# bioinformatics-centre/kaiju

Measured on NVIDIA H100. Metric: reads/sec (150 bp paired, MEM mode, synth-viruses .fmi), higher is better.
Workload: dtype int64

## Files before the change

kaiju_b200/csrc/kj_build.h:

```cpp
#pragma once

#define KJ_BLD_THREADS 256
struct KjBuildLcode { uint8_t v[256]; };

template <int RB>
__global__ void __launch_bounds__(KJ_BLD_THREADS) kj_bld_count(const uint8_t* __restrict__ bwt, const __grid_constant__ KjBuildLcode lc, uint64_t n, uint32_t rep, int alen,
                                                                uint32_t* __restrict__ tile_counts) {
    __shared__ uint32_t tot[KJ_MAX_ALEN];
    __shared__ uint8_t lcs[256];
    __shared__ uint8_t cnt[KJ_MAX_ALEN * KJ_BLD_THREADS];
    if (threadIdx.x < KJ_MAX_ALEN) tot[threadIdx.x] = 0;
    lcs[threadIdx.x] = lc.v[threadIdx.x];
    for (int a = 0; a < KJ_MAX_ALEN; a++) cnt[a * KJ_BLD_THREADS + threadIdx.x] = 0;
    __syncthreads();
    const uint64_t tile_rows = (uint64_t)KJ_BLD_THREADS * RB, start = (uint64_t)blockIdx.x * tile_rows;
    for (uint32_t i = threadIdx.x; i < tile_rows; i += KJ_BLD_THREADS) {
        const uint64_t row = start + i;
        if (row < n) cnt[(uint32_t)lcs[bwt[rep == 1 ? row : row / rep]] * KJ_BLD_THREADS + threadIdx.x]++;
    }
    for (int a = 0; a < alen; a++) {
        uint32_t v = cnt[a * KJ_BLD_THREADS + threadIdx.x];
        for (int m = 16; m > 0; m >>= 1) v += __shfl_xor_sync(0xffffffffu, v, m);
        if ((threadIdx.x & 31) == 0 && v) atomicAdd(&tot[a], v);
    }
// ... 40 lines not shown
            #pragma unroll
            for (int x = 0; x < 16; x++) {
                const uint32_t m = __vcmpeq4(mine[q * 16 + x], a4) & 0x01010101u;
                bits |= (uint64_t)((m * 0x01020408u) >> 24) << (4 * x);
            }
            w[q] = bits; c += (uint32_t)__popcll(bits);
        }
        uint32_t x = c;
        for (int d = 1; d < 32; d <<= 1) { const uint32_t o = __shfl_up_sync(0xffffffffu, x, d); if (lane >= (uint32_t)d) x += o; }
        if (lane == 31) wsum[wid] = x;
        __syncthreads();
        uint32_t base = 0;
        for (uint32_t k = 0; k < wid; k++) base += wsum[k];
        __syncthreads();
        if (b < nb) {
            uint64_t hdr = Cdev[a] + tile_prefix[(uint64_t)blockIdx.x * KJ_MAX_ALEN + a] + (uint64_t)(base + x - c);
            uint64_t* rec = rank + ((uint64_t)a * nb + b) * RW;
            if (RW == 2) { *(ulonglong2*)rec = make_ulonglong2(hdr, w[0]); }
            else {
                const uint64_t p1 = (uint64_t)__popcll(w[0]), p2 = p1 + (uint64_t)__popcll(w[RB / 64 > 1 ? 1 : 0]);
                hdr = (hdr & KJ_CNT_MASK) | (p1 << KJ_P1_SHIFT) | (p2 << KJ_P2_SHIFT);
                *(ulonglong2*)rec = make_ulonglong2(hdr, w[0]);
                *(ulonglong2*)(rec + 2) = make_ulonglong2(w[RB / 64 > 1 ? 1 : 0], w[RB / 64 > 2 ? 2 : 0]);
            }
        }
    }
}
__global__ void kj_bld_letters(const uint8_t* __restrict__ bwt, const __grid_constant__ KjBuildLcode lc, uint64_t n, uint32_t rep, uint64_t nwords, uint64_t* __restrict__ letters) {
    __shared__ uint8_t lcs[256];
    lcs[threadIdx.x] = lc.v[threadIdx.x];
    __syncthreads();
    for (uint64_t wd = (uint64_t)blockIdx.x * blockDim.x + threadIdx.x; wd < nwords; wd += (uint64_t)gridDim.x * blockDim.x) {
        uint64_t v = 0;
        for (int t = 0; t < KJ_LETTERS_PER_WORD; t++) { const uint64_t row = wd * KJ_LETTERS_PER_WORD + t; if (row < n) v |= (uint64_t)lcs[bwt[rep == 1 ? row : row / rep]] << (5 * t); }
        letters[wd] = v;
    }
}
__global__ void kj_bld_sa_tax(const uint8_t* __restrict__ sa, uint64_t n_entries, uint64_t first, int nbytes, int pbits, uint32_t nseq, const uint32_t* __restrict__ seq_tax,
                              uint32_t* __restrict__ sa_tax, uint32_t* __restrict__ err) {
    for (uint64_t e = (uint64_t)blockIdx.x * blockDim.x + threadIdx.x; e < n_entries; e += (uint64_t)gridDim.x * blockDim.x) {
        const uint8_t* p = sa + e * (uint64_t)nbytes; uint64_t val = 0;
        for (int b = 0; b < nbytes; b++) val = (val << 8) + p[b];
        const uint64_t seq = val >> pbits;
        if (seq >= nseq) { atomicOr(err, 64u); continue; }
        sa_tax[first + e] = seq_tax[seq];
    }
}
template <class IdxT>
__global__ void kj_bld_sa_tax_scaled(const KjDevIndex* __restrict__ base_ix, uint64_t n_entries, int64_t bias, int exp, uint64_t n_rows, uint32_t rep, uint32_t* __restrict__ sa_tax) {
    for (uint64_t e = (uint64_t)blockIdx.x * blockDim.x + threadIdx.x; e < n_entries; e += (uint64_t)gridDim.x * blockDim.x) {
        const uint64_t k = (uint64_t)((int64_t)e + bias) << exp;
        sa_tax[e] = k < n_rows ? kj_sa_taxon<IdxT>(*base_ix, k / rep) : KJ_TAX_BAD;
    }
}
__global__ void kj_bld_repeat_u32(const uint32_t* __restrict__ src, uint64_t n_out, uint32_t rep, uint32_t* __restrict__ dst) {
    for (uint64_t i = (uint64_t)blockIdx.x * blockDim.x + threadIdx.x; i < n_out; i += (uint64_t)gridDim.x * blockDim.x) dst[i] = src[i / rep];
}
template <class IdxT>
static __device__ __forceinline__ uint64_t kj_bld_rank(const KjDevIndex& ix, uint32_t c, uint64_t k) {
    uint64_t v = (uint64_t)kj_rank<IdxT>(ix, c, (IdxT)k);
    if (k >= ix.quirk_lo) v -= ix.quirk_d[c];
    return v;
}
template <class IdxT>
__global__ void kj_bld_quirk(const KjDevIndex* __restrict__ ix, uint64_t k, uint64_t* __restrict__ quirk_d) {
    const uint32_t a = threadIdx.x;
    if (a < (uint32_t)ix->alen) quirk_d[a] = (uint64_t)kj_rank<IdxT>(*ix, a, (IdxT)k) - ix->C[a];
}
template <class IdxT>
__global__ void kj_bld_kmer_level(const KjDevIndex* __restrict__ ix, const KjKmer* __restrict__ cur, uint64_t n_cur, KjKmer* __restrict__ nxt) {
    for (uint64_t t = (uint64_t)blockIdx.x * blockDim.x + threadIdx.x; t < n_cur * 20u; t += (uint64_t)gridDim.x * blockDim.x) {
        const KjKmer iv = cur[t / 20u]; const uint32_t a = (uint32_t)(t % 20u); KjKmer o; o.lo = 0; o.hi = 0;
        if (iv.lo < iv.hi) { o.lo = kj_bld_rank<IdxT>(*ix, a + 1u, iv.lo); o.hi = kj_bld_rank<IdxT>(*ix, a + 1u, iv.hi); if (o.lo >= o.hi) { o.lo = 0; o.hi = 0; } }
        nxt[t] = o;
    }
}
__global__ void kj_bld_kmer_narrow(const KjKmer* __restrict__ src, uint64_t n, KjKmer32* __restrict__ dst) {
    for (uint64_t t = (uint64_t)blockIdx.x * blockDim.x + threadIdx.x; t < n; t += (uint64_t)gridDim.x * blockDim.x) { dst[t].lo = (uint32_t)src[t].lo; dst[t].hi = (uint32_t)src[t].hi; }
}

static int kj_bld_upload(void* d, const void* h, size_t bytes) {
    const size_t CH = (size_t)1 << 30;
    for (size_t o = 0; o < bytes; o += CH) CK(cudaMemcpy((char*)d + o, (const char*)h + o, std::min(CH, bytes - o), cudaMemcpyHostToDevice));
    return KJ_OK;
}

static int kj_device_build(kj_ctx* c, const kj_index_view& v, const uint8_t lcode[256], uint32_t rep, const kj_ctx* base, uint64_t& tot) {
    KjHostIndex& H = c->H; const int alen = H.alen; const uint64_t n = H.bwtlen, nb = H.nb; const int wide = H.wide;
    const uint32_t RB = kj_rank_rows(wide), RW = kj_rank_words(wide);
    KjBuildLcode lc; memcpy(lc.v, lcode, 256);
    const int grid_big = c->sm_count * 16;
    KjDevBuf bwt; int rc = bwt.grow((size_t)v.bwtlen); if (rc) return rc;
    const uint8_t* d_bwt = bwt.as<uint8_t>();
    if ((rc = kj_bld_upload(bwt.p, v.bwt, (size_t)v.bwtlen))) return rc;
    const uint64_t ntiles = (nb + KJ_BLD_THREADS - 1) / KJ_BLD_THREADS;
    if (ntiles >= (1ull << 31)) { kj_err() = "index too large"; return KJ_ERR_UNSUPPORTED; }
    KjDevBuf tc, tp, small;
    if ((rc = tc.grow(ntiles * KJ_MAX_ALEN * 4)) || (rc = tp.grow(ntiles * KJ_MAX_ALEN * 8)) || (rc = small.grow(3 * KJ_MAX_ALEN * 8 + 64))) return rc;
    uint32_t* d_tc = tc.as<uint32_t>(); uint64_t* d_tp = tp.as<uint64_t>();
    uint64_t* d_tot = small.as<uint64_t>(); uint64_t* d_C = d_tot + KJ_MAX_ALEN + 1;
    if (wide) kj_bld_count<KJ_RANK_ROWS_WIDE><<<(unsigned)ntiles, KJ_BLD_THREADS>>>(d_bwt, lc, n, rep, alen, d_tc);
    else kj_bld_count<KJ_RANK_ROWS_NARROW><<<(unsigned)ntiles, KJ_BLD_THREADS>>>(d_bwt, lc, n, rep, alen, d_tc);
    kj_bld_scan_tiles<<<1, 32 * KJ_MAX_ALEN>>>(d_tc, ntiles, d_tp, d_tot);
    CK(cudaGetLastError());
    uint64_t tots[KJ_MAX_ALEN]; CK(cudaMemcpy(tots, d_tot, sizeof tots, cudaMemcpyDeviceToHost));
    H.C[0] = 0; for (int a = 0; a < alen; a++) H.C[a + 1] = H.C[a] + tots[a];
// ... 39 lines not shown
            const uint64_t m = std::min(CHE, n_sa - e0);
            CK(cudaMemcpy(sa.p, v.sa + e0 * (uint64_t)v.nbytes, (size_t)m * (size_t)v.nbytes, cudaMemcpyHostToDevice));
            kj_bld_sa_tax<<<grid_big, 256>>>(sa.as<uint8_t>(), m, e0, v.nbytes, v.pbits, (uint32_t)v.nseq, c->seq_tax.as<uint32_t>(), c->sa_tax.as<uint32_t>(), d_err);
            if (c->sa_acc.p) kj_bld_sa_tax<<<grid_big, 256>>>(sa.as<uint8_t>(), m, e0, v.nbytes, v.pbits, (uint32_t)v.nseq, c->seq_acc.as<uint32_t>(), c->sa_acc.as<uint32_t>(), d_err);
            CK(cudaGetLastError()); CK(cudaDeviceSynchronize()); c->launches++;
        }
        uint32_t e = 0; CK(cudaMemcpy(&e, d_err, 4, cudaMemcpyDeviceToHost));
        if (e & 64u) { CK(cudaMemset(d_err, 0, 4)); kj_err() = "corrupt suffix array (sequence number out of range)"; return KJ_ERR_IO; }
    } else {
        const int64_t last = (int64_t)((n - 1) >> H.sa_exp) - H.sa_bias;
        n_sa = last >= 0 ? (uint64_t)last + 1 : 0;
        if ((rc = c->sa_tax.grow(std::max<size_t>(n_sa * 4, 16)))) return rc;
        tot += std::max<size_t>(n_sa * 4, 16);
        if (base->H.wide) kj_bld_sa_tax_scaled<uint64_t><<<grid_big, 256>>>(base->ix.as<KjDevIndex>(), n_sa, H.sa_bias, H.sa_exp, n, rep, c->sa_tax.as<uint32_t>());
        else kj_bld_sa_tax_scaled<uint32_t><<<grid_big, 256>>>(base->ix.as<KjDevIndex>(), n_sa, H.sa_bias, H.sa_exp, n, rep, c->sa_tax.as<uint32_t>());
        CK(cudaGetLastError()); CK(cudaDeviceSynchronize()); c->launches++;
    }
    c->n_sa = n_sa;
    return KJ_OK;
}

static int kj_device_build_kmer(kj_ctx* c, int k, uint64_t& tot, KjDevBuf& dst, int& k_out) {
    KjHostIndex& H = c->H; const int wide = H.wide; const KjDevIndex* ix = c->ix.as<KjDevIndex>();
    if (H.quirk_lo != ~0ull && &dst == &c->kmer) {
        if (wide) kj_bld_quirk<uint64_t><<<1, 32>>>(ix, H.bwtlen - 65536ull, c->quirk.as<uint64_t>()); else kj_bld_quirk<uint32_t><<<1, 32>>>(ix, H.bwtlen - 65536ull, c->quirk.as<uint64_t>());
        CK(cudaGetLastError()); CK(cudaMemcpy(H.quirk_d, c->quirk.p, sizeof H.quirk_d, cudaMemcpyDeviceToHost)); c->launches++;
    }
    k_out = 0;
    if (k < 2 || k > 7 || H.alen != 21) return KJ_OK;
    uint64_t n_final = 1; for (int d = 0; d < k; d++) n_final *= 20;
    { size_t fr = 0, to = 0; CK(cudaMemGetInfo(&fr, &to));
      while (k > 2 && (double)n_final * (2.0 * sizeof(KjKmer) + sizeof(KjKmer32)) > 0.8 * (double)fr) { k--; n_final /= 20; } }
    KjDevBuf a, b; int rc;
    if ((rc = a.grow(n_final * sizeof(KjKmer))) || (rc = b.grow(n_final * sizeof(KjKmer)))) return rc;
    std::vector<KjKmer> first(20); for (uint32_t l = 0; l < 20; l++) { first[l].lo = H.C[l + 1]; first[l].hi = H.C[l + 2]; }
    CK(cudaMemcpy(a.p, first.data(), 20 * sizeof(KjKmer), cudaMemcpyHostToDevice));
    uint64_t n_cur = 20;
    for (int d = 1; d < k; d++) {
        const unsigned g = (unsigned)std::min<uint64_t>((n_cur * 20 + 255) / 256, (uint64_t)c->sm_count * 32);
        if (wide) kj_bld_kmer_level<uint64_t><<<g, 256>>>(ix, a.as<KjKmer>(), n_cur, b.as<KjKmer>()); else kj_bld_kmer_level<uint32_t><<<g, 256>>>(ix, a.as<KjKmer>(), n_cur, b.as<KjKmer>());
        CK(cudaGetLastError()); c->launches++;
        std::swap(a, b); n_cur *= 20;
    }
    if (wide) { dst = std::move(a); tot += n_final * sizeof(KjKmer); }
    else {
        if ((rc = dst.grow(n_final * sizeof(KjKmer32)))) return rc;
        tot += n_final * sizeof(KjKmer32);
        kj_bld_kmer_narrow<<<c->sm_count * 8, 256>>>(a.as<KjKmer>(), n_final, dst.as<KjKmer32>()); CK(cudaGetLastError()); c->launches++;
    }
    CK(cudaDeviceSynchronize());
    k_out = k;
    return KJ_OK;
}
```

kaiju_b200/csrc/kj_core.h:

```cpp
#pragma once
#include "kj_warp.h"
#include "kj_layout.h"

#define KJ_SEG_CAP(max_frag) ((max_frag) / 4u + 8u)
struct KjKept { uint64_t lo; uint32_t len; uint32_t aux; };

struct KjSmemLayout {
    uint32_t qkey_off, qpay_off, kept_off, res_off, res2_off, pre_off, ids_off, qord_off, aa_off, aa_stride, frag_off, hflag_off,
             segcnt_off, seghist_off, accs_off, total, segs_off;
#if defined(KJ_EMU)
    uint32_t guard[16], nguard;
#endif
};
#if defined(KJ_EMU)
#define KJ_GUARD(L, o) { (L).guard[(L).nguard++] = (o); (o) += 64u; }
#else
#define KJ_GUARD(L, o)
#endif
static KJ_HD uint32_t kj_align(uint32_t x, uint32_t a) { return (x + a - 1) / a * a; }
static KJ_HD KjSmemLayout kj_smem_layout(const KjRunParams& p) {
    KjSmemLayout L; uint32_t o = 0;
#if defined(KJ_EMU)
    L.nguard = 0;
#endif
// ... 41 lines not shown
};
static KJ_DEV void kj_flag_error(KjWarpCtx& cx, uint32_t bit) {
#if defined(KJ_EMU)
    *cx.err |= bit;
#else
    atomicOr(cx.err, bit);
#endif
}

static KJ_DEV uint64_t kj_ld64(const void* p) {
#if defined(KJ_EMU)
    return *(const uint64_t*)p;
#else
    uint64_t v; asm volatile("ld.global.nc.u64 %0, [%1];" : "=l"(v) : "l"(p)); return v;
#endif
}
static KJ_DEV void kj_ld128(const void* p, uint64_t& a, uint64_t& b) {
#if defined(KJ_EMU)
    a = ((const uint64_t*)p)[0]; b = ((const uint64_t*)p)[1];
#else
    asm volatile("ld.global.nc.v2.u64 {%0, %1}, [%2];" : "=l"(a), "=l"(b) : "l"(p));
#endif
}
template <class IdxT>
static KJ_DEV IdxT kj_rank_at(const uint64_t* base, IdxT k) {
    if (sizeof(IdxT) == 4) {
        uint64_t h, wd; kj_ld128(base + 2u * (size_t)((uint32_t)k >> 6), h, wd);
        return (IdxT)((uint32_t)h + (uint32_t)kj_popcll(wd & ((1ull << ((uint32_t)k & 63u)) - 1ull)));
    }
    const uint32_t q = (uint32_t)((uint64_t)k >> 6), blk = q / 3u, wi = q - 3u * blk, bit = (uint32_t)k & 63u;
    const uint64_t* rec = base + 4u * (size_t)blk;
    const uint64_t hdr = kj_ld64(rec);
    const uint64_t ww = kj_ld64(rec + 1u + wi);
    const uint32_t pc = (uint32_t)kj_popcll(ww & ((1ull << bit) - 1ull));
    const uint32_t add = wi == 0 ? 0u : ((uint32_t)(hdr >> (32u + 8u * wi)) & 0xffu);
    return (IdxT)((hdr & KJ_CNT_MASK) + (uint64_t)(add + pc));
}
static KJ_DEV const uint64_t* kj_letter_base(const KjDevIndex& ix, uint32_t c) { return ix.rank_base[c]; }
template <class IdxT>
static KJ_DEV IdxT kj_rank(const KjDevIndex& ix, uint32_t c, IdxT k) { return kj_rank_at<IdxT>(kj_letter_base(ix, c), k); }
template <class IdxT>
static KJ_DEV bool kj_update_si(const KjDevIndex& ix, uint32_t c, IdxT& lo, IdxT& hi) {
    const uint64_t* base = kj_letter_base(ix, c);
    IdxT nlo = kj_rank_at<IdxT>(base, lo), nhi = kj_rank_at<IdxT>(base, hi);
    if (sizeof(IdxT) == 8) { if (hi >= (IdxT)ix.quirk_lo) { const IdxT d = (IdxT)ix.quirk_d[c]; nhi -= d; if (lo >= (IdxT)ix.quirk_lo) nlo -= d; } }
    if (nlo >= nhi) return false;
    lo = nlo; hi = nhi; return true;
}
static KJ_DEV int kj_hibit64(uint64_t x) { uint32_t h = (uint32_t)(x >> 32); return h ? 63 - kj_clz(h) : 31 - kj_clz((uint32_t)x); }
static KJ_DEV uint32_t kj_letter(const KjDevIndex& ix, uint64_t k) {
    uint64_t wd = k / KJ_LETTERS_PER_WORD; uint32_t s = (uint32_t)(k - wd * KJ_LETTERS_PER_WORD) * 5u;
    return (uint32_t)(ix.letters[wd] >> s) & 31u;
}
template <class IdxT>
static KJ_DEV uint64_t kj_sa_locate(const KjDevIndex& ix, uint64_t k, bool& is_seq) {
    uint32_t c = 1;
    KJ_ROLLED
    while (c != 0 && (k & ix.sa_check)) { c = kj_letter(ix, k); const bool q = k >= ix.quirk_lo; k = (uint64_t)kj_rank<IdxT>(ix, c, (IdxT)k); if (q) k -= ix.quirk_d[c]; }
    is_seq = c == 0;
    return is_seq ? k : (uint64_t)((int64_t)(k >> ix.sa_exp) - ix.sa_bias);
}
template <class IdxT>
static KJ_DEV uint32_t kj_sa_taxon(const KjDevIndex& ix, uint64_t k) {
    bool is_seq; const uint64_t e = kj_sa_locate<IdxT>(ix, k, is_seq);
    return is_seq ? ix.seq_tax[e] : ix.sa_tax[e];
}

#define KJ_PHASE_A_LETTERS 9
#define KJ_ST_OPEN 0
#define KJ_ST_EXACT 1
#define KJ_ST_KDEAD 2
template <class IdxT> struct KjChain { IdxT lo, hi; int i; int st; };
#if defined(KJ_EMU)
struct KjEmuStats { unsigned long long rounds, round_steps, lane_steps, chains, blocks, lookaheads, pops_frag, pops_var, var_steps, var_pushed; };
extern thread_local KjEmuStats kj_emu_stats;
#endif

template <class IdxT>
static KJ_DEV void kj_chain_start(const KjDevIndex& ix, const uint8_t* frag, int j, uint32_t Lmin, KjChain<IdxT>& ch) {
    const int k = ix.kmer_k; int i = j; int budget = KJ_PHASE_A_LETTERS - 1;
    ch.st = KJ_ST_OPEN;
    if (k > 0 && j >= k && Lmin >= (uint32_t)k) {
        uint32_t idx = 0;
        KJ_ROLLED
        for (int t = 0; t < k; t++) idx = idx * 20u + (uint32_t)(frag[j - t] - 1u);
        IdxT lo, hi;
        if (sizeof(IdxT) == 4) { const KjKmer32 e = ((const KjKmer32*)ix.kmer)[idx]; lo = (IdxT)e.lo; hi = (IdxT)e.hi; }
        else { const KjKmer e = ((const KjKmer*)ix.kmer)[idx]; lo = (IdxT)e.lo; hi = (IdxT)e.hi; }
        if (lo >= hi) { ch.lo = 0; ch.hi = 0; ch.i = j + 1; ch.st = KJ_ST_KDEAD; return; }
        ch.lo = lo; ch.hi = hi; i = j - k + 1; budget = KJ_PHASE_A_LETTERS - k;
    } else {
        const uint32_t c = frag[j]; ch.lo = (IdxT)ix.C[c]; ch.hi = (IdxT)ix.C[c + 1];
    }
    KJ_ROLLED
    while (i > 0 && budget > 0) { if (!kj_update_si<IdxT>(ix, frag[i - 1], ch.lo, ch.hi)) { ch.st = KJ_ST_EXACT; break; } i--; budget--; }
    if (i == 0) ch.st = KJ_ST_EXACT;
    ch.i = i;
}
template <class IdxT>
static KJ_DEV void kj_chain_finish(const KjDevIndex& ix, const uint8_t* frag, KjChain<IdxT>& ch) {
    int i = ch.i;
    KJ_ROLLED
    while (i > 0) { if (!kj_update_si<IdxT>(ix, frag[i - 1], ch.lo, ch.hi)) break; i--; }
    ch.i = i; ch.st = KJ_ST_EXACT;
}
template <class IdxT>
static KJ_DEV void kj_finish_selected(const Warp& w, const KjDevIndex& ix, const uint8_t* frag, bool sel, KjChain<IdxT>& ch) {
#if defined(KJ_EMU)
    const int i0 = ch.i;
#endif
    if (sel) kj_chain_finish<IdxT>(ix, frag, ch);
    w.sync();
#if defined(KJ_EMU)
    { const uint32_t st = sel ? (uint32_t)(i0 - ch.i) + 1u : 0u; const uint32_t mx = warp_max_u32(w, st); const uint32_t nsel = (uint32_t)kj_popc(w.ballot(sel));
      uint32_t sum = st; for (int m = 16; m > 0; m >>= 1) sum += w.shfl_xor(sum, m);
      if (w.lane == 0) { kj_emu_stats.rounds++; kj_emu_stats.round_steps += mx; kj_emu_stats.lane_steps += sum; kj_emu_stats.chains += nsel; } }
#endif
}

template <class IdxT>
static KJ_DEV int kj_chain_lbval(const KjChain<IdxT>& ch, int j, int kk) { return ch.st == KJ_ST_EXACT ? ch.i : (j - kk + 2 > 0 ? j - kk + 2 : 0); }
template <class IdxT>
static KJ_DEV int kj_chain_lb(const Warp& w, const KjChain<IdxT>& ch, bool ran, int j, int kk, int lb_ext) {
    const uint32_t inf = w.ballot(ran && ch.st != KJ_ST_OPEN);
    const uint32_t below = w.lane < 31 ? inf & ~((2u << w.lane) - 1u) : 0u;
    const int v = w.shfl(kj_chain_lbval<IdxT>(ch, j, kk), below ? kj_ffs(below) - 1 : 0);
    return below ? v : lb_ext;
}
template <class IdxT>
// ... 417 lines not shown
        }
    }
    return nsegs;
}
KJ_NOINLINE int kj_seg_regions(const KjSegArgs A, int n) {
    KjSeg* segs = A.segs;
    int ns = kj_seg_level<0>(A, 0, n, segs, 0);
    A.w.sync();
    if (ns > 1) {
        if (A.w.lane == 0) {
            int cur = ns - 1, nx = cur - 1;
            KJ_ROLLED
            while (nx >= 0) {
                if (segs[cur].begin - segs[nx].end - 1 < 0) {
                    if (segs[cur].end < segs[nx].end) segs[cur].end = segs[nx].end;
                    if (segs[cur].begin > segs[nx].begin) segs[cur].begin = segs[nx].begin;
                    segs[nx].begin = -1;
                } else cur = nx;
                nx--;
            }
            int o = 0;
            KJ_ROLLED
            for (int t = 0; t < ns; t++) if (segs[t].begin >= 0) segs[o++] = segs[t];
            segs[ns].begin = o;
        }
        A.w.sync();
        ns = segs[ns].begin;
        A.w.sync();
    }
    return ns;
}
static KJ_DEV int kj_seg(KjWarpCtx& cx, int n, const bool compact) {
    if (n < KJ_SEG_WINDOW) return 0;
    if (!kj_seg_flags(cx, n, compact)) return 0;
    KjSegArgs A; A.w = cx.w; A.frag = cx.smem + cx.L.frag_off; A.hf = cx.smem + cx.L.hflag_off; A.segs = (KjSeg*)(cx.smem + cx.L.segs_off);
    A.scratch = cx.smem + cx.L.segcnt_off; A.lnf = cx.ix->lnfact; A.cap = (int)KJ_SEG_CAP(cx.rp->max_frag); A.err = cx.err;
    return kj_seg_regions(A, n);
}

static KJ_DEV KjKept* kj_kept_ptr(KjWarpCtx& cx, uint32_t idx) {
    if (idx < cx.rp->kept_cap_smem) return (KjKept*)(cx.smem + cx.L.kept_off) + idx;
    uint32_t s = idx - cx.rp->kept_cap_smem;
    if (s >= cx.rp->scratch_entries) { kj_flag_error(cx, 2u); s = cx.rp->scratch_entries - 1; }
    return cx.spill + s;
}

struct KjIdsArgs { Warp w; const KjDevIndex* ix; const KjKept* kept_smem; const KjKept* spill; uint32_t kept_cap, spill_cap; uint32_t* ids; uint32_t* accs; };
template <class IdxT>
KJ_NOINLINE uint64_t kj_ids_and_lca_fn(const KjIdsArgs A, uint32_t nkept) {
    const Warp& w = A.w; const KjDevIndex& ix = *A.ix;
    uint32_t* ids = A.ids;
    uint32_t nids = 0, nacc = 0;
    uint32_t* accs = A.accs;
    KJ_ROLLED
    for (uint32_t e = 0; e < nkept && nids <= 20; e++) {
        const uint32_t se = e - A.kept_cap;
        const KjKept kk = e < A.kept_cap ? A.kept_smem[e] : A.spill[se < A.spill_cap ? se : A.spill_cap - 1];
        KJ_ROLLED
        for (uint32_t base = 0; base < kk.len && nids <= 20; base += 32) {
            uint32_t t = base + (uint32_t)w.lane; bool act = t < kk.len;
            uint32_t tax = KJ_TAX_BAD, acc = 0xffffffffu;
            if (act) { bool is_seq; const uint64_t en = kj_sa_locate<IdxT>(ix, kk.lo + t, is_seq); tax = is_seq ? ix.seq_tax[en] : ix.sa_tax[en]; if (accs) acc = is_seq ? ix.seq_acc[en] : ix.sa_acc[en]; }
            uint32_t nact = kk.len - base < 32u ? kk.len - base : 32u;
            KJ_ROLLED
            for (uint32_t s = 0; s < nact && nids <= 20; s++) {
                uint32_t id = w.shfl(tax, (int)s);
                if (id == KJ_TAX_BAD) continue;
                if (accs) {
                    const uint32_t a = w.shfl(acc, (int)s);
                    if (a != 0xffffffffu && nacc < 20u) { const bool dupa = (uint32_t)w.lane < nacc && accs[w.lane] == a; if (!w.any(dupa)) { if (w.lane == 0) accs[nacc] = a; nacc++; w.sync(); } }
                }
                bool dup = (uint32_t)w.lane < nids && ids[w.lane] == id;
                if (!w.any(dup)) { if (w.lane == 0) ids[nids] = id; nids++; w.sync(); }
            }
        }
    }
    if (accs && w.lane == 0) accs[20] = nacc;
    const uint64_t hi = (uint64_t)nids << 32;
    if (nids == 0) return hi | KJ_TAX_BAD;
    w.sync();
    if (nids == 1) return hi | ids[0];
    uint32_t id = (uint32_t)w.lane < nids ? ids[w.lane] : KJ_TAX_BAD;
    uint32_t depth = id != KJ_TAX_BAD ? ix.tax_depth[id] : 0u;
    bool present = depth > 0;
    uint32_t pm = w.ballot(present);
    if (!pm) return hi | KJ_TAX_BAD;
    uint32_t shallow = warp_min_u32(w, present ? depth : 0xffffffffu);
    if (present) for (uint32_t d = depth; d > shallow; d--) id = ix.tax_parent[id];
    int first = kj_ffs(pm) - 1;
    KJ_ROLLED
    for (uint32_t guard = 0; guard <= shallow + 1; guard++) {
        uint32_t f = w.shfl(id, first);
        bool diff = present && id != f;
        if (!w.any(diff)) return hi | f;
        if (present) id = ix.tax_parent[id];
    }
    return hi | KJ_TAX_BAD;
}
template <class IdxT>
static KJ_DEV uint32_t kj_ids_and_lca(KjWarpCtx& cx, uint32_t nkept) {
    KjIdsArgs A; A.w = cx.w; A.ix = cx.ix; A.kept_smem = (const KjKept*)(cx.smem + cx.L.kept_off); A.spill = cx.spill;
    A.kept_cap = cx.rp->kept_cap_smem; A.spill_cap = cx.rp->scratch_entries; A.ids = (uint32_t*)(cx.smem + cx.L.ids_off);
    A.accs = cx.want_acc ? (uint32_t*)(cx.smem + cx.L.accs_off) : nullptr;
    const uint64_t r = kj_ids_and_lca_fn<IdxT>(A, nkept);
    cx.nids = (uint32_t)(r >> 32);
    return (uint32_t)r;
}


static KJ_DEV bool kj_seg_gate(KjWarpCtx& cx, KjQueue& q, uint32_t arr, uint32_t start, uint32_t len, bool greedy) {
    int ns = kj_seg(cx, (int)len, greedy);
    if (ns == 0) return false;
    kj_queue_make_dirty(cx, q);
    const KjSeg* segs = (const KjSeg*)(cx.smem + cx.L.segs_off);
    const uint8_t* frag = cx.smem + cx.L.frag_off; const KjTables& tb = *cx.tb;
    uint32_t st = 0;
    KJ_ROLLED
    for (int s = 0; s <= ns; s++) {
        int plen = (s < ns ? segs[s].begin : (int)len) - (int)st;
        if (plen > (int)cx.rp->m) {
            uint32_t val = (uint32_t)plen; bool ok = true;
            if (greedy) { uint32_t sc = 0; for (int t = 0; t < plen; t++) { uint32_t a = frag[st + t]; sc += (uint32_t)tb.b62[a][a]; } val = sc; ok = sc >= cx.rp->min_score; }
            kj_queue_emit(cx, q, cx.w.lane == 0 && ok, val, KJ_ORDER_LATE + q.late, kj_qpay(arr, true, start + 3u * st, (uint32_t)plen));
            if (ok) q.late++;
        }
        if (s < ns) st = (uint32_t)segs[s].end + 1u;
    }
// ... 213 lines not shown
```

kaiju_b200/csrc/kj_device.cu:

```cuda
#include <cuda_runtime.h>
#include <algorithm>
#include <chrono>
#include <cmath>
#include <cstdio>
#include <cstdlib>
#include <cstring>
#include <map>
#include <memory>
#include <mutex>
#include <string>
#include <thread>
#include <vector>
#include "kj_core.h"
#include "kj_core_greedy.h"
#include "kj_host.h"

#define KJ_WARPS_PER_CTA 8
#define KJ_MIN_BLOCKS 4
#define KJ_MIN_BLOCKS_GREEDY_SPLIT 4
#define KJ_MIN_BLOCKS_GREEDY 4
#define KJ_CLAIM 4
#define KJ_CHUNK_READS (1u << 20)
#define KJ_CHUNK_BYTES (1ull << 28)

// ... 116 lines not shown
    if ((threadIdx.x & 31) == 0) atomicMax(out, m);
}

__global__ void kj_count_kernel(const uint64_t* __restrict__ taxon, uint64_t n, const uint64_t* __restrict__ tax_id, uint32_t n_present, uint32_t n_tax,
                                unsigned long long* __restrict__ counts) {
    for (uint64_t r = (uint64_t)blockIdx.x * blockDim.x + threadIdx.x; r < n; r += (uint64_t)gridDim.x * blockDim.x) {
        const uint64_t id = taxon[r]; uint32_t slot = n_tax;
        if (id) {
            uint32_t lo = 0, hi = n_present;
            while (lo < hi) { const uint32_t mid = (lo + hi) >> 1; if (tax_id[mid] < id) lo = mid + 1; else hi = mid; }
            if (lo < n_present && tax_id[lo] == id) slot = lo;
            else { lo = n_present; hi = n_tax; while (lo < hi) { const uint32_t mid = (lo + hi) >> 1; if (tax_id[mid] < id) lo = mid + 1; else hi = mid; } if (lo < n_tax && tax_id[lo] == id) slot = lo; }
        }
        atomicAdd(counts + slot, 1ull);
    }
}
__global__ void kj_count_commit(unsigned long long* __restrict__ total, unsigned long long* __restrict__ pending, uint32_t n) {
    for (uint32_t i = blockIdx.x * blockDim.x + threadIdx.x; i < n; i += gridDim.x * blockDim.x) { total[i] += pending[i]; pending[i] = 0; }
}

struct KjDevBuf {
    void* p = nullptr; size_t cap = 0;
    KjDevBuf() = default;
    KjDevBuf(const KjDevBuf&) = delete; KjDevBuf& operator=(const KjDevBuf&) = delete;
    KjDevBuf(KjDevBuf&& o) noexcept : p(o.p), cap(o.cap) { o.p = nullptr; o.cap = 0; }
    KjDevBuf& operator=(KjDevBuf&& o) noexcept { if (this != &o) { reset(); p = o.p; cap = o.cap; o.p = nullptr; o.cap = 0; } return *this; }
    ~KjDevBuf() { reset(); }
    void reset() { if (p) cudaFree(p); p = nullptr; cap = 0; }
    int grow(size_t need, size_t alloc) {
        if (need <= cap) return KJ_OK;
        reset(); void* q = nullptr; CK(cudaMalloc(&q, alloc)); p = q; cap = alloc; return KJ_OK;
    }
    int grow(size_t need) { return grow(need, need); }
    template <class T> T* as() const { return (T*)p; }
};

struct KjSlot {
    KjDevBuf seq[2], off[2];
    KjDevBuf tax, best, ids, nids, acc, nacc, frag, fraglen;
    KjDevBuf spill, gscratch, ws;
    cudaStream_t stream = nullptr, fstream = nullptr;
    cudaEvent_t ev_in = nullptr, ev_f[2] = {nullptr, nullptr}, ev_s[2] = {nullptr, nullptr};
};

struct KjFilesState; static void kj_files_state_free(KjFilesState* S);
struct kj_ctx {
    std::unique_ptr<KjFilesState, void (*)(KjFilesState*)> files{nullptr, kj_files_state_free};
    int device = 0; kj_params params{}; int sm_count = 0;
    KjHostIndex H;
    KjDevIndex dix{};
    KjDevBuf ix, tables;
    KjDevBuf ix_mem, kmer_mem; int kmer_k_mem = 0;
    KjDevBuf rank, letters, sa_tax, seq_tax, sa_acc, seq_acc, tax_parent, tax_depth, tax_id, lnfact, kmer;
    uint64_t index_bytes = 0; uint64_t n_sa = 0; double build_ms = 0.0;
    KjDevBuf counter, err, maxlen, quirk;
    KjDevBuf evbreaks; uint32_t n_evbreaks = 0;
    KjDevBuf counts, counts_pending; uint32_t n_counts = 0, n_present = 0;
    uint32_t variant_boost = 1;
    KjDevBuf prep;
    KjSlot slot[2];
    cudaEvent_t ev_a = nullptr, ev_b = nullptr;
    uint64_t launches = 0; double last_kernel_ms = 0.0;
    int grid = 0; size_t smem_bytes = 0; KjKernel grid_kernel = nullptr;
};

struct KjOut {
    uint64_t* tax = nullptr; uint32_t* best = nullptr; uint32_t* compact = nullptr;
    uint64_t* ids = nullptr; uint8_t* nids = nullptr;
    uint32_t* acc = nullptr; uint8_t* nacc = nullptr;
    char* frag = nullptr; uint32_t frag_stride = 0; uint32_t* fraglen = nullptr;
    unsigned long long* counts = nullptr;
};

template <class T> static int upload(const std::vector<T>& v, KjDevBuf& d, uint64_t& total) {
    size_t bytes = std::max<size_t>(v.size() * sizeof(T), 16);
    int rc = d.grow(bytes); if (rc) return rc;
    if (!v.empty()) CK(cudaMemcpy(d.p, v.data(), v.size() * sizeof(T), cudaMemcpyHostToDevice));
    total += bytes; return KJ_OK;
}

#define KJ_SMEM_WS_LIMIT (75u * 1024u)
static bool kj_use_fixed(const KjRunParams& rp) {
    if (rp.ws_global || rp.mode != 1) return false;
    const KjSmemLayout a = kj_smem_layout(rp), b = kj_smem_layout(kj_fixed_profile(rp.mode));
    return memcmp(&a, &b, sizeof a) == 0 && rp.max_len == 152 && rp.kept_cap_smem == KJ_KEPT_SMEM;
}
static int configure_launch(kj_ctx* c, KjKernel front, KjKernel kern, size_t smem) {
    {
        static std::mutex attr_mu; static std::map<std::pair<int, KjKernel>, size_t> attr_set;
        std::lock_guard<std::mutex> lk(attr_mu);
        for (KjKernel k : {front, kern}) {
            if (!k) continue;
            size_t& cur = attr_set[{c->device, k}];
            if (smem > cur) { CK(cudaFuncSetAttribute(k, cudaFuncAttributeMaxDynamicSharedMemorySize, (int)smem)); cur = smem; }
        }
    }
    if (kern == c->grid_kernel && smem == c->smem_bytes && c->grid > 0) return KJ_OK;
    int per_sm = 0; CK(cudaOccupancyMaxActiveBlocksPerMultiprocessor(&per_sm, kern, KJ_WARPS_PER_CTA * 32, smem));
    if (per_sm < 1) { kj_err() = "kernel does not fit on an SM"; return KJ_ERR_UNSUPPORTED; }
    c->grid = c->sm_count * per_sm;
    c->grid_kernel = kern; c->smem_bytes = smem;
    return KJ_OK;
}

static int upload_evalue_breaks(kj_ctx* c) {
    c->evbreaks.reset(); c->n_evbreaks = 0;
    std::vector<double> br; int rc = kj_build_evalue_breaks(c->params, c->H.db_length, br); if (rc) return rc;
    if (br.empty()) return KJ_OK;
    if ((rc = c->evbreaks.grow(br.size() * sizeof(double)))) return rc;
    CK(cudaMemcpy(c->evbreaks.p, br.data(), br.size() * sizeof(double), cudaMemcpyHostToDevice));
    c->n_evbreaks = (uint32_t)br.size();
    return KJ_OK;
}

static thread_local bool kj_transient_ctx = false;
static int new_ctx(kj_ctx** out, int device, const kj_params* params) {
    int rc = kj_check_params(*params); if (rc) return rc;
    int ndev = 0;
    if (cudaGetDeviceCount(&ndev) != cudaSuccess || ndev <= 0) { kj_err() = "no CUDA device available (this library has no CPU fallback)"; return KJ_ERR_NO_DEVICE; }
    if (device < 0 || device >= ndev) { kj_err() = "device ordinal out of range"; return KJ_ERR_ARG; }
    CK(cudaSetDevice(device));
    kj_ctx* c = new kj_ctx(); c->device = device; c->params = *params;
    std::unique_ptr<kj_ctx, void (*)(kj_ctx*)> guard(c, kj_destroy);
    cudaDeviceProp prop; CK(cudaGetDeviceProperties(&prop, device)); c->sm_count = prop.multiProcessorCount;
    if ((rc = c->err.grow(sizeof(uint32_t)))) return rc;
    CK(cudaMemset(c->err.p, 0, sizeof(uint32_t)));
    if ((rc = c->quirk.grow(sizeof c->H.quirk_d))) return rc;
    CK(cudaMemset(c->quirk.p, 0, sizeof c->H.quirk_d));
    *out = guard.release(); return KJ_OK;
}
static int upload_descriptor(kj_ctx* c) {
    KjHostIndex& H = c->H; KjDevIndex& D = c->dix; memset(&D, 0, sizeof D);
    D.rank = c->rank.as<const uint64_t>(); D.nb = H.nb; D.letters = c->letters.as<const uint64_t>(); D.bwtlen = H.bwtlen; D.alen = H.alen;
    for (int a = 0; a <= H.alen; a++) D.C[a] = H.C[a];
    for (int a = 0; a < H.alen; a++) D.rank_base[a] = D.rank + (uint64_t)a * H.nb * kj_rank_words(H.wide);
    D.sa_acc = c->sa_acc.as<const uint32_t>(); D.seq_acc = c->seq_acc.as<const uint32_t>();
    D.sa_tax = c->sa_tax.as<const uint32_t>(); D.seq_tax = c->seq_tax.as<const uint32_t>(); D.sa_check = H.sa_check; D.sa_exp = H.sa_exp; D.sa_bias = H.sa_bias;
    D.n_sa = c->n_sa; D.nseq = H.nseq;
    D.tax_parent = c->tax_parent.as<const uint32_t>(); D.tax_depth = c->tax_depth.as<const uint32_t>(); D.tax_id = c->tax_id.as<const uint64_t>(); D.n_tax = (uint32_t)H.tax_id.size();
    D.lnfact = c->lnfact.as<const double>(); D.n_lnfact = (int)H.lnfact.size(); D.kmer = H.kmer_k ? c->kmer.p : nullptr; D.kmer_k = H.kmer_k; D.wide = H.wide; D.tables = c->tables.as<KjTables>();
    D.quirk_lo = H.quirk_lo; D.mono = H.quirk_lo == ~0ull ? 1 : 0; D.quirk_d = c->quirk.as<uint64_t>();
    int rc = c->ix.grow(sizeof(KjDevIndex)); if (rc) return rc;
    CK(cudaMemcpy(c->ix.p, &D, sizeof(KjDevIndex), cudaMemcpyHostToDevice));
    if (c->kmer_mem.p && c->kmer_k_mem) {
        KjDevIndex M = D; M.kmer = c->kmer_mem.p; M.kmer_k = c->kmer_k_mem;
        if ((rc = c->ix_mem.grow(sizeof(KjDevIndex)))) return rc;
        CK(cudaMemcpy(c->ix_mem.p, &M, sizeof(KjDevIndex), cudaMemcpyHostToDevice));
    }
    return KJ_OK;
}
static int upload_small(kj_ctx* c, uint64_t& tot) {
    KjHostIndex& H = c->H; int rc;
    if ((rc = upload(H.tax_parent, c->tax_parent, tot)) || (rc = upload(H.tax_depth, c->tax_depth, tot)) || (rc = upload(H.tax_id, c->tax_id, tot)) || (rc = upload(H.lnfact, c->lnfact, tot)) ||
        (rc = c->tables.grow(sizeof(KjTables)))) return rc;
    CK(cudaMemcpy(c->tables.p, &H.tables, sizeof(KjTables), cudaMemcpyHostToDevice));
    return KJ_OK;
}
static int finish_ctx(kj_ctx* c, uint64_t tot) {
    KjHostIndex& H = c->H; int rc;
    CK(cudaMemcpy(c->quirk.p, H.quirk_d, sizeof H.quirk_d, cudaMemcpyHostToDevice));
    if ((rc = upload_descriptor(c))) return rc;
    c->index_bytes = tot;
    if ((rc = c->counter.grow(4 * sizeof(unsigned long long))) || (rc = c->maxlen.grow(2 * sizeof(unsigned int)))) return rc;
    for (KjSlot& S : c->slot) {
        CK(cudaStreamCreateWithFlags(&S.stream, cudaStreamNonBlocking)); CK(cudaStreamCreateWithFlags(&S.fstream, cudaStreamNonBlocking));
        CK(cudaEventCreateWithFlags(&S.ev_in, cudaEventDisableTiming));
        for (int b = 0; b < 2; b++) { CK(cudaEventCreateWithFlags(&S.ev_f[b], cudaEventDisableTiming)); CK(cudaEventCreateWithFlags(&S.ev_s[b], cudaEventDisableTiming)); }
    }
    CK(cudaEventCreate(&c->ev_a)); CK(cudaEventCreate(&c->ev_b));
    if ((rc = upload_evalue_breaks(c))) return rc;
    c->n_counts = (uint32_t)H.tax_id.size() + 1u; c->n_present = H.n_present;
    if ((rc = c->counts.grow((size_t)c->n_counts * 8)) || (rc = c->counts_pending.grow((size_t)c->n_counts * 8))) return rc;
    CK(cudaMemset(c->counts.p, 0, (size_t)c->n_counts * 8)); CK(cudaMemset(c->counts_pending.p, 0, (size_t)c->n_counts * 8));
    return KJ_OK;
}

template <class Fill> static int create_ctx(kj_ctx** out, int device, const kj_params* params, Fill fill) {
    kj_ctx* c = nullptr; int rc = new_ctx(&c, device, params); if (rc) return rc;
    std::unique_ptr<kj_ctx, void (*)(kj_ctx*)> guard(c, kj_destroy);
    rc = fill(c->H); if (rc) return rc;
    KjHostIndex& H = c->H; uint64_t tot = 0;
    c->n_sa = H.sa_tax.size(); H.sa_tax.push_back(KJ_TAX_BAD);
    if (!H.seq_acc.empty()) { H.sa_acc.push_back(0xffffffffu); if ((rc = upload(H.sa_acc, c->sa_acc, tot)) || (rc = upload(H.seq_acc, c->seq_acc, tot))) return rc; }
    if ((rc = upload(H.rank, c->rank, tot)) || (rc = upload(H.letters, c->letters, tot)) || (rc = upload(H.sa_tax, c->sa_tax, tot)) ||
        (rc = upload(H.seq_tax, c->seq_tax, tot)) || (rc = upload_small(c, tot)) || (rc = (H.wide ? upload(H.kmer, c->kmer, tot) : upload(H.kmer32, c->kmer, tot)))) return rc;
    std::vector<uint64_t>().swap(H.rank); std::vector<uint64_t>().swap(H.letters); std::vector<uint32_t>().swap(H.sa_tax); std::vector<KjKmer>().swap(H.kmer); std::vector<KjKmer32>().swap(H.kmer32);
    if ((rc = finish_ctx(c, tot))) return rc;
    *out = guard.release(); return KJ_OK;
}

#include "kj_build.h"
static int create_ctx_device(kj_ctx** out, int device, const kj_params* params, const kj_index_view& v, const kj_taxonomy_view& t, uint32_t copies, const kj_ctx* base) {
    kj_ctx* c = nullptr; int rc = new_ctx(&c, device, params); if (rc) return rc;
    std::unique_ptr<kj_ctx, void (*)(kj_ctx*)> guard(c, kj_destroy);
    const auto t0 = std::chrono::steady_clock::now();
    uint8_t lcode[256]; rc = kj_build_host_meta(v, t, copies, c->H, lcode); if (rc) return rc;
    uint64_t tot = 0;
    if ((rc = upload_small(c, tot)) || (rc = kj_device_build(c, v, lcode, copies, base, tot))) return rc;
    c->H.kmer_k = 0;
    if ((rc = upload_descriptor(c))) return rc;
    { const char* ek = getenv("KJ_KMER_K"); if ((rc = kj_device_build_kmer(c, ek ? atoi(ek) : kj_default_kmer_k(c->H.bwtlen), tot, c->kmer, c->H.kmer_k))) return rc; }
    if (!c->H.wide && c->H.kmer_k == 6 && !kj_transient_ctx && !getenv("KJ_KMER_K") && !getenv("KJ_NO_KMER7")) {
        size_t fr = 0, to = 0; CK(cudaMemGetInfo(&fr, &to));
        if ((double)fr > 1.28e9 * (2.0 * sizeof(KjKmer) + sizeof(KjKmer32)) + 16e9 && (rc = kj_device_build_kmer(c, 7, tot, c->kmer_mem, c->kmer_k_mem))) return rc;
    }
    std::vector<uint32_t>().swap(c->H.seq_tax);
    if ((rc = finish_ctx(c, tot))) return rc;
    CK(cudaDeviceSynchronize());
    c->build_ms = std::chrono::duration<double, std::milli>(std::chrono::steady_clock::now() - t0).count();
    *out = guard.release(); return KJ_OK;
}

extern "C" int kj_create(kj_ctx** out, int device, const kj_params* params, const kj_index_view* index, const kj_taxonomy_view* taxonomy) {
    if (!out || !params || !index || !taxonomy) { kj_err() = "kj_create: null argument"; return KJ_ERR_ARG; }
// ... 332 lines not shown
```

kaiju_b200/csrc/kj_layout.h:

```cpp
#pragma once
#include <stdint.h>

#define KJ_RANK_ROWS_NARROW 64
#define KJ_RANK_ROWS_WIDE 192
#define KJ_RANK_WORDS_NARROW 2
#define KJ_RANK_WORDS_WIDE 4
static inline uint32_t kj_rank_rows(int wide) { return wide ? KJ_RANK_ROWS_WIDE : KJ_RANK_ROWS_NARROW; }
static inline uint32_t kj_rank_words(int wide) { return wide ? KJ_RANK_WORDS_WIDE : KJ_RANK_WORDS_NARROW; }
#define KJ_LETTERS_PER_WORD 12
#define KJ_MAX_ALEN 24
#define KJ_MAX_IDS 21
#define KJ_MAX_BEST_SI 20
#define KJ_TAX_BAD 0xffffffffu
#define KJ_MAX_MM 8
#define KJ_SEG_WINDOW 12
#define KJ_KEPT_SMEM 20

#define KJ_CNT_MASK 0xffffffffffull
#define KJ_P1_SHIFT 40
#define KJ_P2_SHIFT 48

struct KjKmer { uint64_t lo, hi; };
struct KjKmer32 { uint32_t lo, hi; };

struct KjTables {
    uint8_t codon_aa[64];
    int8_t b62[KJ_MAX_ALEN][KJ_MAX_ALEN];
    uint8_t subst[KJ_MAX_ALEN][20];
    int32_t seg_logfix[KJ_SEG_WINDOW + 1];
    int32_t seg_locut_fix, seg_hicut_fix;
    char letters[KJ_MAX_ALEN];
    uint8_t aa_index[32];
};

struct KjDevIndex {
    const uint64_t* rank; uint64_t nb;
    const uint64_t* rank_base[KJ_MAX_ALEN];
    const uint64_t* letters;
    uint64_t bwtlen; int alen;
    uint64_t C[KJ_MAX_ALEN + 1];
    const uint32_t* sa_tax; const uint32_t* seq_tax;
    const uint32_t* sa_acc; const uint32_t* seq_acc;
    uint64_t sa_check; int sa_exp; int64_t sa_bias; uint64_t n_sa; uint32_t nseq;
    const uint32_t* tax_parent; const uint32_t* tax_depth; const uint64_t* tax_id; uint32_t n_tax;
    const double* lnfact; int n_lnfact;
    const void* kmer; int kmer_k;
    int wide;
    int mono;
    uint64_t quirk_lo; const uint64_t* quirk_d;
    const KjTables* tables;
};

struct KjRunParams {
    int mode;
    uint32_t m, e, min_score, seed_length;
    int use_evalue, seg, protein, name_mode;
    const double* ev_breaks; uint32_t n_ev_breaks;
    uint32_t max_len;
    uint32_t max_frag;
    uint32_t item_cap;
    uint32_t kept_cap_smem;
    uint32_t scratch_entries;
    uint32_t variant_cap;
    uint32_t ws_global;
};
```

Before: 50.34 million.

## Precompute per-row taxon table and pack SA-locate waves across kept intervals

Builds a dense row_tax array (one taxon per BWT row) at index load time when the index is narrow and enough device memory is free, so read classification can replace the iterative LF-walk suffix-array locate with a single global load. The id-collection loop is also restructured so that short kept intervals are packed together into full 32-lane warp waves using a prefix scan, instead of each interval using only part of the warp. The cost is 4 bytes per BWT row of device memory, extra build time, and more complex warp bookkeeping. The accession path still falls back to the locate walk.

```diff
diff --git a/kaiju_b200/csrc/kj_build.h b/kaiju_b200/csrc/kj_build.h
--- a/kaiju_b200/csrc/kj_build.h
+++ b/kaiju_b200/csrc/kj_build.h
@@ -116,6 +116,9 @@
         const uint64_t k = (uint64_t)((int64_t)e + bias) << exp;
         sa_tax[e] = k < n_rows ? kj_sa_taxon<IdxT>(*base_ix, k / rep) : KJ_TAX_BAD;
     }
+}
+__global__ void kj_bld_row_tax(const KjDevIndex* __restrict__ ix, uint64_t n_rows, uint32_t* __restrict__ row_tax) {
+    for (uint64_t k = (uint64_t)blockIdx.x * blockDim.x + threadIdx.x; k < n_rows; k += (uint64_t)gridDim.x * blockDim.x) row_tax[k] = kj_row_taxon<uint32_t>(*ix, k);
 }
 __global__ void kj_bld_repeat_u32(const uint32_t* __restrict__ src, uint64_t n_out, uint32_t rep, uint32_t* __restrict__ dst) {
     for (uint64_t i = (uint64_t)blockIdx.x * blockDim.x + threadIdx.x; i < n_out; i += (uint64_t)gridDim.x * blockDim.x) dst[i] = src[i / rep];
@@ -261,3 +264,17 @@
     k_out = k;
     return KJ_OK;
 }
+
+#define KJ_ROW_TAX_MARGIN (8ull << 30)
+static int kj_device_build_row_tax(kj_ctx* c, uint64_t& tot) {
+    const KjHostIndex& H = c->H;
+    if (H.wide || kj_transient_ctx) return KJ_OK;
+    const size_t bytes = (size_t)H.bwtlen * 4;
+    size_t fr = 0, to = 0; CK(cudaMemGetInfo(&fr, &to));
+    if (bytes + KJ_ROW_TAX_MARGIN > fr) return KJ_OK;
+    int rc = c->row_tax.grow(bytes); if (rc) return rc;
+    kj_bld_row_tax<<<c->sm_count * 16, 256>>>(c->ix.as<KjDevIndex>(), H.bwtlen, c->row_tax.as<uint32_t>());
+    CK(cudaGetLastError()); CK(cudaDeviceSynchronize()); c->launches++;
+    tot += bytes;
+    return KJ_OK;
+}
diff --git a/kaiju_b200/csrc/kj_core.h b/kaiju_b200/csrc/kj_core.h
--- a/kaiju_b200/csrc/kj_core.h
+++ b/kaiju_b200/csrc/kj_core.h
@@ -117,11 +117,21 @@
     uint64_t wd = k / KJ_LETTERS_PER_WORD; uint32_t s = (uint32_t)(k - wd * KJ_LETTERS_PER_WORD) * 5u;
     return (uint32_t)(ix.letters[wd] >> s) & 31u;
 }
+#if defined(KJ_EMU)
+struct KjEmuStats { unsigned long long rounds, round_steps, lane_steps, chains, blocks, lookaheads, pops_frag, pops_var, var_steps, var_pushed,
+                                       id_reads, kept, sa_waves, sa_lf_steps, sa_dep_steps; };
+extern thread_local KjEmuStats kj_emu_stats;
+#endif
 template <class IdxT>
 static KJ_DEV uint64_t kj_sa_locate(const KjDevIndex& ix, uint64_t k, bool& is_seq) {
     uint32_t c = 1;
     KJ_ROLLED
-    while (c != 0 && (k & ix.sa_check)) { c = kj_letter(ix, k); const bool q = k >= ix.quirk_lo; k = (uint64_t)kj_rank<IdxT>(ix, c, (IdxT)k); if (q) k -= ix.quirk_d[c]; }
+    while (c != 0 && (k & ix.sa_check)) {
+        c = kj_letter(ix, k); const bool q = k >= ix.quirk_lo; k = (uint64_t)kj_rank<IdxT>(ix, c, (IdxT)k); if (q) k -= ix.quirk_d[c];
+#if defined(KJ_EMU)
+        kj_emu_stats.sa_lf_steps++;
+#endif
+    }
     is_seq = c == 0;
     return is_seq ? k : (uint64_t)((int64_t)(k >> ix.sa_exp) - ix.sa_bias);
 }
@@ -130,16 +140,14 @@
     bool is_seq; const uint64_t e = kj_sa_locate<IdxT>(ix, k, is_seq);
     return is_seq ? ix.seq_tax[e] : ix.sa_tax[e];
 }
+template <class IdxT>
+static KJ_DEV uint32_t kj_row_taxon(const KjDevIndex& ix, uint64_t k) { return k < ix.C[1] ? KJ_TAX_BAD : kj_sa_taxon<IdxT>(ix, k); }
 
 #define KJ_PHASE_A_LETTERS 9
 #define KJ_ST_OPEN 0
 #define KJ_ST_EXACT 1
 #define KJ_ST_KDEAD 2
 template <class IdxT> struct KjChain { IdxT lo, hi; int i; int st; };
-#if defined(KJ_EMU)
-struct KjEmuStats { unsigned long long rounds, round_steps, lane_steps, chains, blocks, lookaheads, pops_frag, pops_var, var_steps, var_pushed; };
-extern thread_local KjEmuStats kj_emu_stats;
-#endif
 
 template <class IdxT>
 static KJ_DEV void kj_chain_start(const KjDevIndex& ix, const uint8_t* frag, int j, uint32_t Lmin, KjChain<IdxT>& ch) {
@@ -663,27 +671,57 @@
     uint32_t* ids = A.ids;
     uint32_t nids = 0, nacc = 0;
     uint32_t* accs = A.accs;
-    KJ_ROLLED
-    for (uint32_t e = 0; e < nkept && nids <= 20; e++) {
-        const uint32_t se = e - A.kept_cap;
-        const KjKept kk = e < A.kept_cap ? A.kept_smem[e] : A.spill[se < A.spill_cap ? se : A.spill_cap - 1];
-        KJ_ROLLED
-        for (uint32_t base = 0; base < kk.len && nids <= 20; base += 32) {
-            uint32_t t = base + (uint32_t)w.lane; bool act = t < kk.len;
-            uint32_t tax = KJ_TAX_BAD, acc = 0xffffffffu;
-            if (act) { bool is_seq; const uint64_t en = kj_sa_locate<IdxT>(ix, kk.lo + t, is_seq); tax = is_seq ? ix.seq_tax[en] : ix.sa_tax[en]; if (accs) acc = is_seq ? ix.seq_acc[en] : ix.sa_acc[en]; }
-            uint32_t nact = kk.len - base < 32u ? kk.len - base : 32u;
-            KJ_ROLLED
-            for (uint32_t s = 0; s < nact && nids <= 20; s++) {
-                uint32_t id = w.shfl(tax, (int)s);
-                if (id == KJ_TAX_BAD) continue;
-                if (accs) {
-                    const uint32_t a = w.shfl(acc, (int)s);
-                    if (a != 0xffffffffu && nacc < 20u) { const bool dupa = (uint32_t)w.lane < nacc && accs[w.lane] == a; if (!w.any(dupa)) { if (w.lane == 0) accs[nacc] = a; nacc++; w.sync(); } }
-                }
-                bool dup = (uint32_t)w.lane < nids && ids[w.lane] == id;
-                if (!w.any(dup)) { if (w.lane == 0) ids[nids] = id; nids++; w.sync(); }
-            }
+    const uint32_t* row_tax = accs ? nullptr : ix.row_tax;
+#if defined(KJ_EMU)
+    if (w.lane == 0) { kj_emu_stats.id_reads++; kj_emu_stats.kept += nkept; }
+#endif
+    auto kept_at = [&](uint32_t x) { const uint32_t sx = x - A.kept_cap; return x < A.kept_cap ? A.kept_smem[x] : A.spill[sx < A.spill_cap ? sx : A.spill_cap - 1]; };
+    uint32_t e = 0, off = 0;
+    KjKept kk; kk.lo = 0; kk.len = 0; kk.aux = 0;
+    if (nkept) kk = kept_at(0);
+    KJ_ROLLED
+    while (e < nkept && nids <= 20) {
+        const uint32_t t = (uint32_t)w.lane, left = kk.len - off;
+        uint64_t row = kk.lo + off + t;
+        uint32_t nact = left < 32u ? left : 32u, next_e = e + (off + nact >= kk.len ? 1u : 0u), next_off = next_e != e ? 0u : off + nact;
+        if (left < 32u && e + 1u < nkept) {
+            const uint32_t x = e + t;
+            uint64_t lo = 0; uint32_t rem = 0;
+            if (x < nkept) { const KjKept kx = kept_at(x); lo = kx.lo; rem = kx.len; if (t == 0) { lo += off; rem -= off; } rem = rem < 33u ? rem : 33u; }
+            uint32_t incl = rem, j = 0;
+            KJ_ROLLED
+            for (int d = 1; d < 32; d <<= 1) { const uint32_t o = w.shfl(incl, w.lane - d); if (w.lane >= d) incl += o; }
+            KJ_ROLLED
+            for (uint32_t s = 16; s > 0; s >>= 1) { if (w.shfl(incl, (int)(j + s - 1)) <= t) j += s; }
+            row = w.shfl64(lo - (uint64_t)(incl - rem), (int)j) + t;
+            const uint32_t total = w.shfl(incl, 31);
+            nact = total < 32u ? total : 32u;
+            const uint32_t nfull = (uint32_t)kj_popc(w.ballot(x < nkept && incl <= 32u));
+            next_e = e + nfull; next_off = 32u - w.shfl(incl, (int)nfull - 1);
+        }
+        uint32_t tax = KJ_TAX_BAD, acc = 0xffffffffu;
+#if defined(KJ_EMU)
+        const unsigned long long lf0 = kj_emu_stats.sa_lf_steps;
+#endif
+        if (t < nact) {
+            if (row_tax) tax = row_tax[row];
+            else { bool is_seq; const uint64_t en = kj_sa_locate<IdxT>(ix, row, is_seq); tax = is_seq ? ix.seq_tax[en] : ix.sa_tax[en]; if (accs) acc = is_seq ? ix.seq_acc[en] : ix.sa_acc[en]; }
+        }
+#if defined(KJ_EMU)
+        { const uint32_t mx = warp_max_u32(w, (uint32_t)(kj_emu_stats.sa_lf_steps - lf0)); if (w.lane == 0) { kj_emu_stats.sa_waves++; kj_emu_stats.sa_dep_steps += mx; } }
+#endif
+        if (next_e != e && next_e < nkept) kk = kept_at(next_e);
+        e = next_e; off = next_off;
+        KJ_ROLLED
+        for (uint32_t s = 0; s < nact && nids <= 20; s++) {
+            uint32_t id = w.shfl(tax, (int)s);
+            if (id == KJ_TAX_BAD) continue;
+            if (accs) {
+                const uint32_t a = w.shfl(acc, (int)s);
+                if (a != 0xffffffffu && nacc < 20u) { const bool dupa = (uint32_t)w.lane < nacc && accs[w.lane] == a; if (!w.any(dupa)) { if (w.lane == 0) accs[nacc] = a; nacc++; w.sync(); } }
+            }
+            bool dup = (uint32_t)w.lane < nids && ids[w.lane] == id;
+            if (!w.any(dup)) { if (w.lane == 0) ids[nids] = id; nids++; w.sync(); }
         }
     }
     if (accs && w.lane == 0) accs[20] = nacc;
diff --git a/kaiju_b200/csrc/kj_device.cu b/kaiju_b200/csrc/kj_device.cu
--- a/kaiju_b200/csrc/kj_device.cu
+++ b/kaiju_b200/csrc/kj_device.cu
@@ -192,6 +192,7 @@
     KjDevBuf ix, tables;
     KjDevBuf ix_mem, kmer_mem; int kmer_k_mem = 0;
     KjDevBuf rank, letters, sa_tax, seq_tax, sa_acc, seq_acc, tax_parent, tax_depth, tax_id, lnfact, kmer;
+    KjDevBuf row_tax;
     uint64_t index_bytes = 0; uint64_t n_sa = 0; double build_ms = 0.0;
     KjDevBuf counter, err, maxlen, quirk;
     KjDevBuf evbreaks; uint32_t n_evbreaks = 0;
@@ -276,7 +277,7 @@
     for (int a = 0; a < H.alen; a++) D.rank_base[a] = D.rank + (uint64_t)a * H.nb * kj_rank_words(H.wide);
     D.sa_acc = c->sa_acc.as<const uint32_t>(); D.seq_acc = c->seq_acc.as<const uint32_t>();
     D.sa_tax = c->sa_tax.as<const uint32_t>(); D.seq_tax = c->seq_tax.as<const uint32_t>(); D.sa_check = H.sa_check; D.sa_exp = H.sa_exp; D.sa_bias = H.sa_bias;
-    D.n_sa = c->n_sa; D.nseq = H.nseq;
+    D.n_sa = c->n_sa; D.row_tax = c->row_tax.as<const uint32_t>(); D.nseq = H.nseq;
     D.tax_parent = c->tax_parent.as<const uint32_t>(); D.tax_depth = c->tax_depth.as<const uint32_t>(); D.tax_id = c->tax_id.as<const uint64_t>(); D.n_tax = (uint32_t)H.tax_id.size();
     D.lnfact = c->lnfact.as<const double>(); D.n_lnfact = (int)H.lnfact.size(); D.kmer = H.kmer_k ? c->kmer.p : nullptr; D.kmer_k = H.kmer_k; D.wide = H.wide; D.tables = c->tables.as<KjTables>();
     D.quirk_lo = H.quirk_lo; D.mono = H.quirk_lo == ~0ull ? 1 : 0; D.quirk_d = c->quirk.as<uint64_t>();
@@ -296,10 +297,11 @@
     CK(cudaMemcpy(c->tables.p, &H.tables, sizeof(KjTables), cudaMemcpyHostToDevice));
     return KJ_OK;
 }
+static int kj_device_build_row_tax(kj_ctx* c, uint64_t& tot);
 static int finish_ctx(kj_ctx* c, uint64_t tot) {
     KjHostIndex& H = c->H; int rc;
     CK(cudaMemcpy(c->quirk.p, H.quirk_d, sizeof H.quirk_d, cudaMemcpyHostToDevice));
-    if ((rc = upload_descriptor(c))) return rc;
+    if ((rc = upload_descriptor(c)) || (rc = kj_device_build_row_tax(c, tot)) || (rc = upload_descriptor(c))) return rc;
     c->index_bytes = tot;
     if ((rc = c->counter.grow(4 * sizeof(unsigned long long))) || (rc = c->maxlen.grow(2 * sizeof(unsigned int)))) return rc;
     for (KjSlot& S : c->slot) {
diff --git a/kaiju_b200/csrc/kj_layout.h b/kaiju_b200/csrc/kj_layout.h
--- a/kaiju_b200/csrc/kj_layout.h
+++ b/kaiju_b200/csrc/kj_layout.h
@@ -37,13 +37,14 @@
     const uint64_t* rank; uint64_t nb;
     const uint64_t* rank_base[KJ_MAX_ALEN];
     const uint64_t* letters;
-    uint64_t bwtlen; int alen;
+    uint64_t bwtlen; int alen; uint32_t nseq;
     uint64_t C[KJ_MAX_ALEN + 1];
     const uint32_t* sa_tax; const uint32_t* seq_tax;
     const uint32_t* sa_acc; const uint32_t* seq_acc;
-    uint64_t sa_check; int sa_exp; int64_t sa_bias; uint64_t n_sa; uint32_t nseq;
-    const uint32_t* tax_parent; const uint32_t* tax_depth; const uint64_t* tax_id; uint32_t n_tax;
-    const double* lnfact; int n_lnfact;
+    uint64_t sa_check; int sa_exp; int64_t sa_bias; uint64_t n_sa;
+    const uint32_t* row_tax;
+    const uint32_t* tax_parent; const uint32_t* tax_depth; const uint64_t* tax_id; uint32_t n_tax; int n_lnfact;
+    const double* lnfact;
     const void* kmer; int kmer_k;
     int wide;
     int mono;
```

Result: faster. 53.57 million, median of 6 (+6.4%).
